# Jiraiya812/Fast-CU-Decision-HEVC

Hardware: AMD Instinct MI355X
Metric: CTUs/sec (RDO decision only) at 4K all-intra (higher is better)
Workload: dtype int32+f64

## Files before the change

### fast-cu-decision-hevc_amd/csrc/fcu_engine.h

```cpp
#pragma once
#include <stdint.h>
#include <string.h>
#include <type_traits>
#include "../../include/fcu.h"

#ifdef FCU_EMU
#include <math.h>
#include <stdio.h>
#include <stdlib.h>
#define FCU_DEV static inline
#define FCU_MEMBER inline
#define FCU_NOINLINE
#define FCU_INLINE
#define FCU_TABLE static const
static int g_emu_phase = 0, g_emu_in_phase = 0, g_emu_lane = 0, g_emu_relax = 0;
#define FCU_EMU_RELAX(on) (g_emu_relax = (on))
static inline int fcu_emu_phase_begin() { g_emu_phase++; g_emu_in_phase = 1; g_emu_lane = 0; return 0; }
static inline int fcu_emu_phase_next(int lane) { if (lane + 1 >= 64) g_emu_in_phase = 0; g_emu_lane = lane + 1; return lane + 1; }
template <class T> static inline T fcu_emu_uni(T v, int site, int line)
{
  enum { SITES = 2048, K = 32, B = 16 };
  struct Seen { int phase, first, cur, idx, n; unsigned char vals[K][B]; };
  static Seen seen[SITES];
  if (g_emu_in_phase && !g_emu_relax && sizeof(T) <= B && site < SITES) {
// ... 3 lines not shown
    if (g_emu_lane == s.first) { if (s.n < K) memcpy(s.vals[s.n++], &v, sizeof(T)); }
    else if (s.idx < s.n && memcmp(s.vals[s.idx], &v, sizeof(T)) != 0) { fprintf(stderr, "FCU_UNI at line %d: value differs between lanes of one phase\n", line); abort(); }
    s.idx++;
  }
  return v;
}
#define FCU_FOR_LANES for (int lane = fcu_emu_phase_begin(); lane < 64; lane = fcu_emu_phase_next(lane))
#define FCU_ATOMIC_ADD(p, v) (*(p) += (v))
#define FCU_ATOMIC_MAX(p, v) do { if (*(p) < (v)) *(p) = (v); } while (0)
#define FCU_ATOMIC_OR(p, v) (*(p) |= (v))
#define FCU_WAVE_ADD(p, v) (*(p) += (v))
#define FCU_WAVE_MIN64(p, v) do { if ((v) < *(p)) *(p) = (v); } while (0)
#define FCU_IN_LDS(p) do { } while (0)
#define FCU_UNI(x) fcu_emu_uni((x), __COUNTER__, __LINE__)
#define FCU_HBM
#define FCU_FLOOR(x) floor(x)
#define FCU_CHECK(c) do { if (!(c)) { fprintf(stderr, "FCU_CHECK failed: %s (line %d)\n", #c, __LINE__); abort(); } } while (0)
static unsigned long long g_emu_cu_paths[3] = { 0, 0, 0 };
#else
#define FCU_DEV __device__ static
#define FCU_MEMBER __device__ inline
#define FCU_NOINLINE __noinline__
#define FCU_INLINE __attribute__((always_inline))
#define FCU_TABLE __device__ static const
#define FCU_FOR_LANES for (int lane = (int)threadIdx.x, fcu_once_ = 1; fcu_once_; fcu_once_ = 0, __syncthreads())
#define FCU_ATOMIC_ADD(p, v) atomicAdd((p), (v))
#define FCU_ATOMIC_MAX(p, v) atomicMax((p), (v))
#define FCU_ATOMIC_OR(p, v) atomicOr((p), (v))
__device__ inline uint32_t fcu_wave_sum(uint32_t v)
{
// ... 17 lines not shown
#define FCU_WAVE_ADD(p, v) do { const uint32_t s_ = fcu_wave_sum(v); if (threadIdx.x == 0) *(p) += s_; } while (0)
#define FCU_WAVE_MIN64(p, v) do { const unsigned long long s_ = fcu_wave_min64(v); if (threadIdx.x == 0 && s_ < *(p)) *(p) = s_; } while (0)
template <class T> __device__ inline T fcu_uni(T v)
{
  static_assert(sizeof(T) % 4 == 0, "dword-sized objects only");
  int w[sizeof(T) / 4];
  __builtin_memcpy(w, &v, sizeof(T));
  for (unsigned i = 0; i < sizeof(T) / 4; i++) w[i] = __builtin_amdgcn_readfirstlane(w[i]);
  __builtin_memcpy(&v, w, sizeof(T));
  return v;
}
#define FCU_UNI(x) fcu_uni(x)
#define FCU_EMU_RELAX(on) do { } while (0)
#if defined(__HIP_DEVICE_COMPILE__)
#define FCU_HBM __attribute__((address_space(1)))
#else
#define FCU_HBM
#endif
#define FCU_GENERIC_(p) ((const __attribute__((address_space(0))) void *)(p))
#define FCU_IN_LDS(p) __builtin_assume(__builtin_amdgcn_is_shared(FCU_GENERIC_(p)))
#define FCU_FLOOR(x) floor(x)
#define FCU_CHECK(c) do { } while (0)
#endif
#define FCU_DIST_ADD(acc, v, e, i, n2) do { \
    if ((n2) >= 64) { (acc) += (uint32_t)((e) * (e)); if (((((i) - lane) + 64) & ((n2) - 1)) == 0) { FCU_WAVE_ADD(&g_S.vc_dist[v], acc); (acc) = 0; } } \
    else FCU_ATOMIC_ADD(&g_S.vc_dist[v], (uint32_t)((e) * (e))); } while (0)
#define FCU_SERIAL FCU_FOR_LANES if (lane == 0)
#if defined(FCU_PROFILE) && !defined(FCU_EMU)
#define FCU_TIC(v) const long long v = clock64()
#ifdef FCU_PROFILE_RQT
#define FCU_QTIC(v) long long v = clock64()
#define FCU_QTOC(E_, v, idx) do { if (threadIdx.x == 0) (E_).C->prof[idx] += (unsigned long long)(clock64() - v); v = clock64(); } while (0)
// ... 4 lines not shown
#define FCU_TOC(E_, v, idx) do { if ((idx) == 10 && threadIdx.x == 0) (E_).C->prof[idx] += (unsigned long long)(clock64() - v); } while (0)
#define FCU_COUNT(E_, idx, n) do { } while (0)
#elif defined(FCU_PROFILE_RDOQ) || defined(FCU_PROFILE_DEPTH)
#define FCU_TOC(E_, v, idx) do { if ((idx) < 11 && threadIdx.x == 0) (E_).C->prof[idx] += (unsigned long long)(clock64() - v); } while (0)
#define FCU_COUNT(E_, idx, n) do { } while (0)
#elif defined(FCU_PROFILE_RMD)
#define FCU_MTOC(E_, v, idx) do { if (threadIdx.x == 0) (E_).C->prof[idx] += (unsigned long long)(clock64() - v); } while (0)
#define FCU_TOC(E_, v, idx) do { if ((idx) < 11 && threadIdx.x == 0) (E_).C->prof[idx] += (unsigned long long)(clock64() - v); } while (0)
#define FCU_COUNT(E_, idx, n) do { } while (0)
#elif defined(FCU_PROFILE_CUSYN)
#define FCU_STOC(E_, v, idx) do { if (threadIdx.x == 0) (E_).C->prof[idx] += (unsigned long long)(clock64() - v); } while (0)
#define FCU_SPATH(E_, path) do { if (threadIdx.x == 0) (E_).C->prof[15] += 1ull << (21 * (path)); } while (0)
#define FCU_S7_COEFF(E_, v, comp) do { if (g_S.prof_s7 == 1) FCU_STOC(E_, v, (comp) ? 14 : 13); } while (0)
#define FCU_TOC(E_, v, idx) do { if ((idx) < 11 && threadIdx.x == 0) (E_).C->prof[idx] += (unsigned long long)(clock64() - v); } while (0)
#define FCU_COUNT(E_, idx, n) do { } while (0)
#else
#define FCU_TOC(E_, v, idx) do { if (threadIdx.x == 0) (E_).C->prof[idx] += (unsigned long long)(clock64() - v); } while (0)
#define FCU_COUNT(E_, idx, n) do { (E_).C->prof[idx] += (unsigned long long)(n); } while (0)
#endif
#else
#define FCU_TIC(v) do { } while (0)
#define FCU_TOC(E_, v, idx) do { } while (0)
#define FCU_COUNT(E_, idx, n) do { } while (0)
#endif
#ifndef FCU_QTOC
#define FCU_QTIC(v) do { } while (0)
#define FCU_QTOC(E_, v, idx) do { } while (0)
#endif
#ifndef FCU_ITOC
#define FCU_ITOC(E_, v, idx) do { } while (0)
#endif
#ifndef FCU_MTOC
#define FCU_MTOC(E_, v, idx) do { } while (0)
#endif
#ifndef FCU_STOC
#define FCU_STOC(E_, v, idx) do { } while (0)
#define FCU_SPATH(E_, path) do { } while (0)
#define FCU_S7_COEFF(E_, v, comp) do { } while (0)
#endif

#include "fcu_tables.h"

struct HotTables { uint32_t bin[256]; uint16_t scan[3][16]; uint8_t scan_cg8[3][4]; uint8_t ctx_ind_map4x4[16]; uint8_t group_idx[32];
                   uint64_t scan4_nib[3], map4_nib; uint32_t cnt_bits[4]; };
#ifdef FCU_EMU
static HotTables g_hot;
#else
__shared__ HotTables g_hot;
// ... 106 lines not shown
  Yuv16 resi_cu, resi_best, qt_resi[4];
  Yuv tmp_pred;
  uint8_t me_pred[9][CTU * CTU];
  int16_t me_h[3][72 * 64];
  int par_ps[4];
  int memo_valid[4][MEMO_K], memo_next[4], memo_zero[4][MEMO_K];
  int16_t memo_mv[4][MEMO_K][NPART][2]; int8_t memo_ref[4][MEMO_K][NPART];
  uint8_t memo_tr_idx[4][MEMO_K][NPART], memo_cbf[4][MEMO_K][3][NPART], memo_tskip[4][MEMO_K][3][NPART];
  alignas(16) int16_t memo_coef[MEMO_K * MEMO_POOL], memo_resi[MEMO_K * MEMO_POOL];
};

struct Env { Chain *C; Scratch *G; int cur_ctu, slice_start; };
struct TU { int log2, tr_depth, part, nparts, x, y, off_y, cw, cwo, cx, cy, c_tr_depth, c_code_all, off_c, cu_depth, plast; };

struct Shared {
  Cabac cab[1 + (MAXDEPTH + 1) + MAXLC + 1];
  uint8_t ref5[5][68]; int dc5[5]; uint32_t cm_dist[5];
  union {
    int16_t lane_abs[MAXLC][32];
    RdoqRec rq_rec[16];
    struct {
      int32_t colsum[128];
      union {
        struct { uint8_t ref[264], reff[264]; };
        uint8_t ref5b[5][68];
      };
    };
  };
  union {
    int16_t rq_lv[16];
    uint32_t sad[36];
// ... 37 lines not shown
  uint64_t lf_frac; uint32_t lf_bins; int lf_valid;
  double dec_j0, dec_j1; int dec_cnt, dec_flip;
#ifdef FCU_PROFILE_CUSYN
  int prof_s7;
#endif
};

enum { CAB_GOON = 0, CAB_CUR0 = 1, CAB_LANE0 = 1 + (MAXDEPTH + 1), CAB_LUMA = CAB_LANE0 + MAXLC };
enum { EST_CODERS = 7 };
static_assert(EST_CODERS * sizeof(Cabac) >= NCTX_INTRA * 2 * sizeof(uint32_t) && EST_CODERS <= MAXLC, "est table does not fit its lane coders");
#define FCU_EST ((uint32_t *)&g_S.cab[CAB_LANE0 + MAXLC - EST_CODERS])
enum { RMD_STAGE_BYTES = 64 * 8 * 2, RMD_COST_BYTES = 35 * 8 };
static_assert(RMD_STAGE_BYTES + RMD_COST_BYTES <= MAXLC * sizeof(Cabac) && (CAB_LANE0 * sizeof(Cabac)) % 8 == 0, "RMD staging does not fit the lane coders");
#define FCU_RMD_STAGE ((int16_t *)&g_S.cab[CAB_LANE0])
#define FCU_RMD_COST ((double *)((char *)&g_S.cab[CAB_LANE0] + RMD_STAGE_BYTES))
FCU_DEV int ref_key(int px, int py, int log2) { return px | (py << 13) | (log2 << 26); }
#ifdef FCU_EMU
static Shared g_S;
#else
__shared__ Shared g_S;
#endif
FCU_DEV Env env_get() { return FCU_UNI(g_S.env); }
FCU_DEV Cabac *slot_ptr(const Env E, int d, int ci) { return ci == CI_CURR_BEST ? &g_S.cab[CAB_CUR0 + d] : &E.G->slots[d][ci]; }


FCU_DEV int part_x(int z) { return (k_z2r[z] & 15) << 2; }
FCU_DEV int part_y(int z) { return (k_z2r[z] >> 4) << 2; }
FCU_DEV int zidx_of(int lx, int ly) { return k_r2z[((ly & 63) >> 2) * 16 + ((lx & 63) >> 2)]; }
FCU_DEV int ilog2(int n) { int l = 0; while ((1 << l) < n) l++; return l; }
FCU_DEV int iabs(int v) { return v < 0 ? -v : v; }
// ... 416 lines not shown
}
FCU_DEV FCU_INLINE int rdoq_signs(const FCU_HBM int32_t *srcg, FCU_HBM int16_t *dstg, int st, int bestLastIdxP1, int lastScanPos)
{
  int absSum = 0;
  for (int sp0 = 0; sp0 < bestLastIdxP1; sp0 += 16) {
    int lv[16]; int32_t sv[16];
#pragma unroll
    for (int k = 0; k < 16; k++) { const int ok = sp0 + k < bestLastIdxP1; lv[k] = ok ? dstg[(sp0 + k) * st] : 0; sv[k] = ok ? srcg[(sp0 + k) * st] : 0; }
#pragma unroll
    for (int k = 0; k < 16; k++) if (sp0 + k < bestLastIdxP1) { absSum += lv[k]; dstg[(sp0 + k) * st] = (int16_t)((sv[k] < 0) ? -lv[k] : lv[k]); }
  }
  for (int sp = bestLastIdxP1; sp <= lastScanPos; sp++) dstg[sp * st] = 0;

  return absSum;
}
FCU_DEV FCU_INLINE void rdoq_sign_hiding(const Params &P, const FCU_HBM int32_t *srcg, FCU_HBM int16_t *dstg, const FCU_HBM RdoqRec *recg, int st, int ch, int bestLastIdxP1, int absSum)
{
  if (P.sign_hiding && absSum >= 2) {
    const long long rdFactor = P.rd_factor[ch];
    int lastCG = -1;
    for (int subSet = (bestLastIdxP1 - 1) >> 4; subSet >= 0; subSet--) {
      const int subPos = subSet << 4; int firstNZ = 16, lastNZ = -1, sum = 0, n;
      uint32_t nzMask = 0, negMask = 0;
      {
        int lv16[16];
#pragma unroll
        for (int k = 0; k < 16; k++) lv16[k] = dstg[(subPos + k) * st];
#pragma unroll
        for (int k = 0; k < 16; k++) { sum += lv16[k]; nzMask |= (uint32_t)(lv16[k] != 0) << k; negMask |= (uint32_t)(lv16[k] < 0) << k; }
      }
      if (nzMask) { lastNZ = 31 - __builtin_clz(nzMask); firstNZ = __builtin_ctz(nzMask); }
// ... 245 lines not shown
template <> struct LaneVar<double> {
  double r = 0;
  __device__ void set(int, double x) { r = x; }
  __device__ double own(int) const { return r; }
  __device__ double get(int k) const
  { union { double d; int i[2]; } u; u.d = r; u.i[0] = FCU_READLANE(u.i[0], k); u.i[1] = FCU_READLANE(u.i[1], k); return u.d; }
  __device__ void put(int k, double x)
  { union { double d; int i[2]; } u, w; u.d = r; w.d = x; u.i[0] = FCU_WRITELANE(w.i[0], k, u.i[0]); u.i[1] = FCU_WRITELANE(w.i[1], k, u.i[1]); r = u.d; }
};
__device__ inline uint32_t lane_mask16(const LaneVar<int> &f) { return (uint32_t)FCU_BALLOT(f.r != 0) & 0xffffu; }
#endif

#ifndef FCU_WAVE_RDOQ_MIN_LOG2
#define FCU_WAVE_RDOQ_MIN_LOG2 2
#endif
FCU_DEV FCU_NOINLINE void rdoq_wave(int c, const int32_t *src, int16_t *dst, int topNZ, int log2, int comp, int scanType, int cbfCtx, const Params &P_, RdoqRec *rec, double *costCGSig)
{
  const Params &P = *FCU_UNI(&P_);
  c = FCU_UNI(c); src = FCU_UNI(src); dst = FCU_UNI(dst); topNZ = FCU_UNI(topNZ); log2 = FCU_UNI(log2); comp = FCU_UNI(comp);
  scanType = FCU_UNI(scanType); cbfCtx = FCU_UNI(cbfCtx); rec = FCU_UNI(rec); costCGSig = FCU_UNI(costCGSig);
  if (topNZ < 0) { FCU_SERIAL { g_S.rw_abs = 0; g_S.rw_lsp = -1; } return; }
  const FCU_HBM int32_t *srcg = (const FCU_HBM int32_t *)src; FCU_HBM int16_t *dstg = (FCU_HBM int16_t *)dst;
  FCU_HBM RdoqRec *recg = (FCU_HBM RdoqRec *)rec; FCU_HBM double *cgg = (FCU_HBM double *)costCGSig;
  auto cb = [&](int ctx, int bin) -> int { return (int)FCU_EST[ctx * 2 + bin]; };
  const int ch = comp ? 1 : 0, N = 1 << log2, n2 = N * N;
  const int qp = comp ? P.qp_c : P.qp;
  const int qbits = rdoq_qbits(log2, qp);
  const double lambda = P.rdoq_lambda[comp];
  const double errScale = P.err_scale[ch][log2 - 2];
  const uint16_t *scan = log2 == 2 ? &g_hot.scan[scanType][0] : k_scan + k_scan_off[scanType * 4 + log2 - 2];
  const uint8_t *scanCG = log2 <= 3 ? g_hot.scan_cg8[log2 == 2 ? 0 : scanType] : k_scan_cg + k_scan_cg_off[scanType * 4 + log2 - 2];
  const int wg = N >> 2, firstSig = first_sig_ctx(log2, scanType, ch);
  const int sigOff = CTX_SIG + (ch ? 28 : 0), cgBase = CTX_SIGCG + (ch ? 2 : 0);
  const uint64_t scan4 = g_hot.scan4_nib[scanType], map4 = g_hot.map4_nib;
  const int cgTop = topNZ >> 4;
  uint64_t cgflag = 0;
  int cgLastScanPos = -1; uint32_t ctxSet = 0; int c1 = 1, c2 = 0;
// ... 349 lines not shown
  int32_t s = 0;
#pragma unroll
  for (int n = 0; n < N; n++) s += (int32_t)(int8_t)(mw[n >> 2] >> (8 * (n & 3))) * (int32_t)a[n];
  return s;
}
template <class F>
FCU_DEV void by_log2(int log2, F f)
{
  switch (log2) {
    case 2: f(std::integral_constant<int, 2>()); break;
    case 3: f(std::integral_constant<int, 3>()); break;
    case 4: f(std::integral_constant<int, 4>()); break;
    default: f(std::integral_constant<int, 5>()); break;
  }
}
template <int LOG2> FCU_DEV const int8_t *basis_row(int useDst, int k) { return (useDst && LOG2 == 2) ? k_dst4 + k * 4 : k_dct + k_dct_off[LOG2 - 2] + (k << LOG2); }
template <int LOG2> FCU_DEV const int8_t *basis_col(int useDst, int n) { return (useDst && LOG2 == 2) ? k_dst4_t + n * 4 : k_dct_t + k_dct_off[LOG2 - 2] + (n << LOG2); }
FCU_DEV int tr_index(int i, int log2) { const int N = 1 << log2; return ((i & (N - 1)) << log2) + (i >> log2); }
template <int LOG2> FCU_DEV int32_t fwd1(const int16_t *resi, int useDst, int idx)
{ constexpr int N = 1 << LOG2, s1 = LOG2 - 1; const int k = idx >> LOG2, y = idx & (N - 1); return (dot_row<N>(basis_row<LOG2>(useDst, k), resi + (y << LOG2)) + (1 << (s1 - 1))) >> s1; }
template <int LOG2> FCU_DEV int32_t fwd2(const int32_t *tmp, int useDst, int idx)
{ constexpr int N = 1 << LOG2, s2 = LOG2 + 6; const int k2 = idx >> LOG2, k1 = idx & (N - 1); return (dot_row<N>(basis_row<LOG2>(useDst, k2), tmp + (k1 << LOG2)) + (1 << (s2 - 1))) >> s2; }
template <int LOG2> FCU_DEV int32_t inv1(const int32_t *deqT, int useDst, int idx)
{ constexpr int N = 1 << LOG2; const int y = idx >> LOG2, kh = idx & (N - 1); return clip3i(-32768, 32767, (dot_row<N>(basis_col<LOG2>(useDst, y), deqT + (kh << LOG2)) + 64) >> 7); }
template <int LOG2> FCU_DEV int32_t inv2(const int32_t *tmp2, int useDst, int idx)
{ constexpr int N = 1 << LOG2; const int y = idx >> LOG2, x = idx & (N - 1); return clip3i(-32768, 32767, (dot_row<N>(basis_col<LOG2>(useDst, x), tmp2 + (y << LOG2)) + 2048) >> 12); }
template <int LOG2> FCU_DEV int32_t fwd1(RowCache<(1 << LOG2), int16_t> &rc, const int16_t *resi, int useDst, int idx)
{ constexpr int N = 1 << LOG2, s1 = LOG2 - 1; const int k = idx >> LOG2, y = idx & (N - 1); return (dot_regs<N>(basis_row<LOG2>(useDst, k), rc.get(resi + (y << LOG2))) + (1 << (s1 - 1))) >> s1; }
template <int LOG2> FCU_DEV int32_t fwd2(RowCache<(1 << LOG2), int32_t> &rc, const int32_t *tmp, int useDst, int idx)
{ constexpr int N = 1 << LOG2, s2 = LOG2 + 6; const int k2 = idx >> LOG2, k1 = idx & (N - 1); return (dot_regs<N>(basis_row<LOG2>(useDst, k2), rc.get(tmp + (k1 << LOG2))) + (1 << (s2 - 1))) >> s2; }
// ... 160 lines not shown
}

FCU_DEV FCU_NOINLINE uint32_t leaf_luma_bits(int c, const CuObj *cu, uint32_t tu_k)
{
  const Env E = env_get(); c = FCU_UNI(c); cu = FCU_UNI(cu); const TU tu = tu_of_key(FCU_UNI(tu_k));
  const int part = tu.part, partSize = cu->part_size[0], log2 = tu.log2;
  cab_reset_bits(c);
  if (part == 0 && E.C->p.slice_type != SLICE_I) { code_skip_flag(E, c, cu, 0); code_pred_mode(c, cu, 0); }
  if (part == 0 && cu->depth[0] == MAXDEPTH) cab_bin(c, partSize == SIZE_2Nx2N, CTX_PARTSIZE);
  if (partSize == SIZE_2Nx2N ? (part == 0) : (tu.tr_depth > 0 && (part & ((cu->nparts >> 2) - 1)) == 0))
    code_luma_dir_bits(c, cu->intra_dir[0][part], g_S.preds);
  if (!(partSize == SIZE_NxN && tu.tr_depth == 0) && log2 != LOG2_MINTU && log2 != min_tu_log2_in_cu(cu->depth[part], cu->part_size[part]))
    cab_bin(c, 0, CTX_SUBDIV + 5 - log2);
  const int cbf = g_S.t_abs > 0;
  cab_bin(c, cbf, CTX_CBF_LUMA + (tu.tr_depth == 0 ? 1 : 0));
  if (cbf) code_coeff_body<1>(c, E.G->p_qscan, 1, g_S.t_lsp, log2, 0, coef_scan_idx(cu->intra_dir[0][part], log2, 0), cu->tskip[0][part], E.C->p, g_S.lane_abs[0]);
  return cab_bits(c);
}

FCU_DEV FCU_NOINLINE void encode_transform(int c, const CuObj *cu, int cuPart, uint32_t root_k, int withLuma)
{
  const Env E = env_get(); c = FCU_UNI(c); cu = FCU_UNI(cu); cuPart = FCU_UNI(cuPart); const TU root = tu_of_key(FCU_UNI(root_k)); withLuma = FCU_UNI(withLuma);
  TU *st = g_S.wk_st; int *ci = g_S.wk_ci; int sp = 0;
  st[0] = root; ci[0] = -1;
  while (sp >= 0) {
    const TU tu = st[sp];
    if (ci[sp] < 0) {
      const int part = cuPart + tu.part, trIdx = tu.tr_depth, subdiv = cu->tr_idx[part] > trIdx;
      if (cu->part_size[part] == SIZE_NxN && trIdx == 0) { }
      else if (tu.log2 > LOG2_MAXTU) { }
      else if (tu.log2 == LOG2_MINTU) { }
// ... 119 lines not shown
  }
}
FCU_DEV FCU_NOINLINE void copy_reco_to_pic(const Yuv *r, int x, int y, int s)
{
  const Env E = env_get(); r = FCU_UNI(r); x = FCU_UNI(x); y = FCU_UNI(y); s = FCU_UNI(s);
  FCU_FOR_LANES {
    for (int c = 0; c < 3; c++) {
      const int sh = c ? 1 : 0, bs = c ? 32 : 64, w = E.C->p.width >> sh, h = E.C->p.height >> sh;
      const uint8_t *src = c == 0 ? r->y : (c == 1 ? r->u : r->v);
      const int px = x >> sh, py = y >> sh, n = s >> sh;
      for (int i = lane; i < n * n; i += 64) { const int yy = i / n, xx = i % n; if (py + yy < h && px + xx < w) E.C->rec[c][(py + yy) * E.C->stride[c] + px + xx] = src[yy * bs + xx]; }
    }
  }
}

FCU_DEV FCU_NOINLINE void tu_trial(CuObj *cu, uint32_t tu_k, int comp, int cab, int save1load2)
{
  const Env E = env_get(); cu = FCU_UNI(cu); const TU tu = tu_of_key(FCU_UNI(tu_k)); comp = FCU_UNI(comp); cab = FCU_UNI(cab); save1load2 = FCU_UNI(save1load2);
  Scratch *G = E.G; const Params &P = E.C->p;
  if (comp && tu.cw == 0) { FCU_SERIAL { g_S.t_dist = 0; g_S.t_abs = 0; g_S.t_lsp = -1; } return; }
  FCU_TIC(t11_);
  const int d = cu->depth_cu, N = comp ? tu.cw : (1 << tu.log2), log2 = ilog2(N), n2 = N * N;
  const int bx = comp ? tu.cx : tu.x, by = comp ? tu.cy : tu.y, bs = comp ? 32 : 64, sh = comp ? 1 : 0;
  const int part = tu.part, layer = LOG2_MAXTU - tu.log2;
  uint8_t *org = yuv_plane(&G->org[d], comp) + by * bs + bx;
  uint8_t *pred = yuv_plane(&G->predt[d], comp) + by * bs + bx;
  uint8_t *recqt = yuv_plane(&G->qt_rec[layer], comp) + by * bs + bx;
  const int px = (cu->x >> sh) + bx, py = (cu->y >> sh) + by;
  uint8_t *recpic = E.C->rec[comp] + py * E.C->stride[comp] + px; const int rs = E.C->stride[comp];
  int16_t *coef = G->qt_coef[comp][layer] + (comp ? tu.off_c : tu.off_y);
  const int useTS = cu->tskip[comp][part];
  const int mode = comp ? chroma_final_mode(cu, part) : cu->intra_dir[0][part];
  const int useDst = comp == 0 && log2 == 2;
  const int qp = comp ? P.qp_c : P.qp;

  if (save1load2 != 2) {
    const int filt = use_filtered_ref(mode, log2, comp == 0);
// ... 13 lines not shown
    FCU_FOR_LANES {
      if (lane == 0) g_S.t_last = -1;
      for (int i = lane; i < n2; i += 64) {
        const int y = i >> log2, x = i & (N - 1); const int v = G->shared_pred[comp][i];
        pred[y * bs + x] = (uint8_t)v; G->p_resi[i] = (int16_t)(org[y * bs + x] - v);
      }
    }
  }
  const int scanType = coef_scan_idx(mode, log2, comp), qbits = rdoq_qbits(log2, qp), qscale = k_quant_scales[qp % 6];
  const uint16_t *iscan = k_iscan + k_scan_off[scanType * 4 + log2 - 2];
  if (useTS) { FCU_FOR_LANES { est_build(cab, lane); for (int i = lane; i < n2; i += 64) { const int sp = iscan[i]; const int32_t ld = level_double((int32_t)G->p_resi[i] << (15 - 8 - log2), qscale, qbits); G->p_lscan[sp] = ld; if (level_nonzero(ld, qbits)) FCU_ATOMIC_MAX(&g_S.t_last, sp); } } }
  else {
    FCU_FOR_LANES { by_log2(log2, [&](auto L) { constexpr int LG = decltype(L)::value; RowCache<(1 << LG), int16_t> rc; for (int i = lane; i < n2; i += 64) G->p_tmp[i] = fwd1<LG>(rc, G->p_resi, useDst, i); }); }
    FCU_FOR_LANES { est_build(cab, lane); by_log2(log2, [&](auto L) { constexpr int LG = decltype(L)::value; RowCache<(1 << LG), int32_t> rc; for (int i = lane; i < n2; i += 64) { const int sp = iscan[i]; const int32_t ld = level_double(fwd2<LG>(rc, G->p_tmp, useDst, i), qscale, qbits); G->p_lscan[sp] = ld; if (level_nonzero(ld, qbits)) FCU_ATOMIC_MAX(&g_S.t_last, sp); } }); }
  }
  {
    FCU_TIC(t8_);
    const int cbfCtx = comp ? (CTX_CBF_CHROMA + tu.tr_depth) : (CTX_CBF_LUMA + (tu.tr_depth == 0 ? 1 : 0));
    const int useRdoq = FCU_UNI((int)(useTS ? P.rdoq_ts : P.rdoq));
    const int onWave = useRdoq && log2 >= FCU_WAVE_RDOQ_MIN_LOG2;
    if (onWave) rdoq_wave(cab, G->p_lscan, G->p_qscan, FCU_UNI(g_S.t_last), log2, comp, scanType, cbfCtx, P, G->r_rec, G->r_cg);
    FCU_FOR_LANES {
      if (comp == 0) for (int i = lane; i < tu.nparts; i += 64) cu->tr_idx[part + i] = (uint8_t)tu.tr_depth;
      if (lane == 0) {
        if (onWave) { g_S.t_abs = g_S.rw_abs; g_S.t_lsp = g_S.rw_lsp; }
        else if (useRdoq) { const RdoqOut o = rdoq<1, 1>(cab, G->p_lscan, G->p_qscan, 1, g_S.t_last, log2, comp, scanType, cbfCtx, P, G->r_rec, G->r_cg); g_S.t_abs = o.abs_sum; g_S.t_lsp = o.last; }
        else { const RdoqOut o = quant_plain(G->p_lscan, G->p_qscan, 1, g_S.t_last, log2, comp, P); g_S.t_abs = o.abs_sum; g_S.t_lsp = o.last; }
        E.C->n_tu_trials++;
        FCU_COUNT(E, 15, (1ull << 40) + (unsigned long long)(g_S.t_last >= 0 ? ((g_S.t_last >> 4) + 1) * 16 : 0));
      }
    }
    FCU_TOC(E, t8_, 8);
  }
  const int absSum = g_S.t_abs;
  FCU_FOR_LANES {
    const int np = comp ? tu_nparts_c(tu) : tu.nparts;
    for (int i = lane; i < np; i += 64) cu->cbf[comp][part + i] = (uint8_t)((absSum > 0 ? 1 : 0) << tu.tr_depth);
    const int cgEnd = ((g_S.t_last >> 4) + 1) << 4;
    const DeqParams dq = deq_params(log2, qp);
    for (int i = lane; i < n2; i += 64) { const int sp = iscan[i]; const int q = (absSum > 0 && sp < cgEnd) ? G->p_qscan[sp] : 0; coef[sp] = (int16_t)q; G->p_tmp[useTS ? i : tr_index(i, log2)] = dequant1(q, dq); }
  }
  if (absSum > 0) {
    if (useTS) { FCU_FOR_LANES { const int s = 15 - 8 - log2; for (int i = lane; i < n2; i += 64) G->p_resi[i] = (int16_t)((G->p_tmp[i] + (1 << (s - 1))) >> s); } }
    else {
      FCU_FOR_LANES { by_log2(log2, [&](auto L) { constexpr int LG = decltype(L)::value; RowCache<(1 << LG), int32_t> rc; for (int i = lane; i < n2; i += 64) G->p_tcoef[i] = inv1<LG>(rc, G->p_tmp, useDst, i); }); }
      FCU_FOR_LANES { by_log2(log2, [&](auto L) { for (int i = lane; i < n2; i += 64) G->p_resi[i] = (int16_t)inv2<decltype(L)::value>(G->p_tcoef, useDst, i); }); }
    }
  }
  FCU_FOR_LANES {
    if (lane == 0) g_S.sad[35] = 0;
  }
  FCU_FOR_LANES {
    uint32_t sse = 0;
    for (int i = lane; i < n2; i += 64) {
      const int y = i >> log2, x = i & (N - 1);
      const int r = clip8(pred[y * bs + x] + (absSum > 0 ? G->p_resi[i] : 0));
      pred[y * bs + x] = (uint8_t)r; recqt[y * bs + x] = (uint8_t)r; recpic[y * rs + x] = (uint8_t)r;
      const int e = org[y * bs + x] - r; sse += (uint32_t)(e * e);
    }
    FCU_WAVE_ADD(&g_S.sad[35], sse);
  }
  FCU_SERIAL { const uint32_t sse = g_S.sad[35]; g_S.t_dist = comp ? (uint32_t)(P.chroma_weight * (double)sse) : sse; }
  FCU_TOC(E, t11_, 11);
}

FCU_DEV FCU_NOINLINE void store_intra_result_qt(uint32_t tu_k, int comp)
{
  const Env E = env_get(); const TU tu = tu_of_key(FCU_UNI(tu_k)); comp = FCU_UNI(comp);
  Scratch *G = E.G;
  if (comp && tu.cw == 0) return;
  const int N = comp ? tu.cw : (1 << tu.log2), layer = LOG2_MAXTU - tu.log2, bs = comp ? 32 : 64, bx = comp ? tu.cx : tu.x, by = comp ? tu.cy : tu.y;
  const int16_t *src = G->qt_coef[comp][layer] + (comp ? tu.off_c : tu.off_y);
  const uint8_t *s = yuv_plane(&G->qt_rec[layer], comp) + by * bs + bx; uint8_t *t = yuv_plane(&G->ts_rec, comp) + by * bs + bx;
  FCU_FOR_LANES { for (int i = lane; i < N * N; i += 64) { G->ts_coef[comp][i] = src[i]; t[(i / N) * bs + (i % N)] = s[(i / N) * bs + (i % N)]; } }
}
FCU_DEV FCU_NOINLINE void load_intra_result_qt(const CuObj *cu, uint32_t tu_k, int comp)
{
// ... 353 lines not shown
}

FCU_DEV FCU_NOINLINE void pu_first_pass_batched(CuObj *cu, uint32_t tu_k)
{
  const Env E = env_get(); cu = FCU_UNI(cu); const TU tu = tu_of_key(FCU_UNI(tu_k));
  Scratch *G = E.G; const Params &P = E.C->p;
  const int d = cu->depth_cu, N = 1 << tu.log2, log2 = tu.log2, n2 = N * N, part = tu.part;
  const int partSize = cu->part_size[part];
  int checkTS = P.transform_skip && log2 == 2;
  if (P.ts_fast) checkTS = checkTS && (partSize == SIZE_NxN);
  const int nc = g_S.n_rd, tsv = checkTS ? 2 : 1, tss = tsv - 1, nvc = nc * tsv;
  FCU_CHECK(nvc <= MAXVC && nvc * n2 <= POOL && (MAXLC % 2) == 0);
  const int qbits = rdoq_qbits(log2, P.qp), qscale = k_quant_scales[P.qp % 6];
  const int useDst = log2 == 2;
  const uint8_t *org = G->org[d].y + tu.y * 64 + tu.x;
  const int haveRefs = FCU_UNI(g_S.ref_tag) == ref_key(cu->x + tu.x, cu->y + tu.y, log2);
  if (!haveRefs) { FCU_TIC(tm_); build_ref(0, cu->x + tu.x, cu->y + tu.y, log2, 1); FCU_MTOC(E, tm_, 14); }
  FCU_FOR_LANES {
    if (lane == 0) g_S.ref_tag = -1;
    const int dc = g_S.dc;
    for (int i = lane; i < nc * n2; i += 64) {
      const int cnd = i / n2, p = i - cnd * n2, y = p >> log2, x = p & (N - 1), mode = g_S.rd_mode[cnd];
      const uint8_t *r = use_filtered_ref(mode, log2, 1) ? g_S.reff : g_S.ref;
      const int v = pred_pixel(r, log2, mode, 1, dc, x, y);
      G->p_pred[i] = (uint8_t)v; G->p_resi[i] = (int16_t)(org[y * 64 + x] - v);
    }
  }
  FCU_FOR_LANES { if (lane < nvc) g_S.vc_last[lane] = -1; by_log2(log2, [&](auto L) { constexpr int LG = decltype(L)::value; RowCache<(1 << LG), int16_t> rc; for (int i = lane; i < nc * n2; i += 64) { const int cnd = i / n2; G->p_tmp[i] = fwd1<LG>(rc, G->p_resi + cnd * n2, useDst, i - cnd * n2); } }); }
  FCU_FOR_LANES {
    est_build(CAB_CUR0 + d, lane);
    by_log2(log2, [&](auto L) { constexpr int LG = decltype(L)::value; RowCache<(1 << LG), int32_t> rc;
      for (int i = lane; i < nvc * n2; i += 64) {
        const int v = i / n2, p = i - v * n2, cnd = (v >> tss), ts = (v & tss);
        const uint16_t *iscan = k_iscan + k_scan_off[coef_scan_idx(g_S.rd_mode[cnd], log2, 0) * 4 + log2 - 2];
        const int32_t t = ts ? ((int32_t)G->p_resi[cnd * n2 + p] << (15 - 8 - log2)) : fwd2<LG>(rc, G->p_tmp + cnd * n2, useDst, p);
        const int sp = iscan[p]; const int32_t ld = level_double(t, qscale, qbits);
        G->p_lscan[sp * nvc + v] = ld;
        if (level_nonzero(ld, qbits)) FCU_ATOMIC_MAX(&g_S.vc_last[v], sp);
      }
    });
  }
  FCU_TIC(t2_);
  FCU_FOR_LANES {
    if (lane < nvc) {
      const int mode = g_S.rd_mode[(lane >> tss)];
      RdoqRec *rrec = G->r_rec + lane; double *rcg = G->r_cg + lane;
      const int cbfCtx = CTX_CBF_LUMA + (tu.tr_depth == 0 ? 1 : 0);
      const RdoqOut o = ((lane & tss) ? P.rdoq_ts : P.rdoq) ? rdoq<0, 1>(CAB_CUR0 + d, G->p_lscan + lane, G->p_qscan + lane, nvc, g_S.vc_last[lane], log2, 0, coef_scan_idx(mode, log2, 0), cbfCtx, P, rrec, rcg)
                                                            : quant_plain(G->p_lscan + lane, G->p_qscan + lane, nvc, g_S.vc_last[lane], log2, 0, P);
      g_S.vc_abs[lane] = o.abs_sum; g_S.vc_lsp[lane] = o.last;
      g_S.vc_dist[lane] = 0;
    }
    if (lane == 0) E.C->n_tu_trials += (unsigned long long)nvc;
  }
  FCU_TOC(E, t2_, 2);
  FCU_FOR_LANES {
    const DeqParams dq = deq_params(log2, P.qp);
    for (int i = lane; i < nvc * n2; i += 64) {
      const int v = i / n2, p = i - v * n2;
      const uint16_t *iscan = k_iscan + k_scan_off[coef_scan_idx(g_S.rd_mode[(v >> tss)], log2, 0) * 4 + log2 - 2];
      const int sp = iscan[p];
      const int q = (g_S.vc_abs[v] > 0 && (sp >> 4) <= (g_S.vc_last[v] >> 4)) ? G->p_qscan[sp * nvc + v] : 0;
      G->p_tmp[((v & tss)) ? i : v * n2 + tr_index(p, log2)] = dequant1(q, dq);
    }
  }
  FCU_FOR_LANES {
    by_log2(log2, [&](auto L) { constexpr int LG = decltype(L)::value; RowCache<(1 << LG), int32_t> rc;
      for (int i = lane; i < nvc * n2; i += 64) {
        const int v = i / n2, p = i - v * n2, ts = (v & tss);
        if (ts) { const int s = 15 - 8 - log2; G->p_tcoef[i] = (G->p_tmp[i] + (1 << (s - 1))) >> s; }
// ... 3 lines not shown
  }
  FCU_FOR_LANES {
    by_log2(log2, [&](auto L) {
      uint32_t acc = 0;
      for (int i = lane; i < nvc * n2; i += 64) {
        const int v = i / n2, p = i - v * n2, cnd = (v >> tss), ts = (v & tss), y = p >> log2, x = p & (N - 1);
        int res = 0;
        if (g_S.vc_abs[v] > 0) res = ts ? (int16_t)G->p_tcoef[i] : inv2<decltype(L)::value>(G->p_tcoef + v * n2, useDst, p);
        const int r = clip8(G->p_pred[cnd * n2 + p] + res);
        G->p_rec[i] = (uint8_t)r;
        const int e = org[y * 64 + x] - r;
        FCU_DIST_ADD(acc, v, e, i, n2);
      }
    });
  }
  FCU_TIC(t3_);
  for (int vbase = 0; vbase < nvc; vbase += MAXLC) {
    const int slotBase = vbase ? (g_S.vc_slot[g_S.pu_best_vc] + 1) % MAXLC : 0;
#if defined(FCU_EMU) && defined(FCU_EMU_TRACE_ROUNDS)
    if (vbase) fprintf(stderr, "second bit-count round: %d variants\n", nvc);
#endif
    FCU_FOR_LANES {
      const int vc = vbase + lane;
      if (lane < MAXLC && vc < nvc) {
        const int cnd = (vc >> tss), ts = (vc & tss), mode = g_S.rd_mode[cnd], cbf = g_S.vc_abs[vc] > 0;
        const int slot = (slotBase + lane) % MAXLC;
        double cost;
        g_S.vc_slot[vc] = (uint8_t)slot;
        if (ts && !cbf) cost = FCU_MAX_DOUBLE;
        else {
// ... 319 lines not shown
  const int d = cu->depth_cu;
  const int N = tu.cw, log2 = ilog2(N), n2 = N * N, trDepth = tu.tr_depth;
  int checkTS = P.transform_skip && N <= 4;
  if (P.ts_fast) {
    checkTS = checkTS && (tu.log2 == 2);
    if (checkTS) { int nb = 0; const int maxp = tu.part + (tu.c_code_all ? 1 : 4); for (int p = tu.part; p < maxp; p++) nb += cu->tskip[0][p]; checkTS = checkTS && (nb > 0); }
  }
  const int tsv = checkTS ? 2 : 1, tss = tsv - 1;
  const int perRound = (tsv == 1 && 10 * n2 <= POOL) ? 2 : 1;
  const int nm = 5 * perRound, nvc = nm * tsv;
  const int qbits = rdoq_qbits(log2, P.qp_c), qscale = k_quant_scales[P.qp_c % 6];
  const int subPart = tu_part_c(tu), nPartsC = tu_nparts_c(tu);
  const int lumaDir = cu->intra_dir[0][tu.part & ~3];
  for (int comp0 = 1; comp0 < 3; comp0 += perRound) {
    const int px = (cu->x >> 1) + tu.cx, py = (cu->y >> 1) + tu.cy;
    for (int cc = 0; cc < perRound; cc++) {
      const int comp = comp0 + cc;
      const uint8_t *org = yuv_plane(&G->org[d], comp) + tu.cy * 32 + tu.cx;
      chroma_leaf_refs5(E, cu, comp, px, py, log2);
      FCU_FOR_LANES {
        for (int i = lane; i < 5 * n2; i += 64) {
          const int m = i / n2, p = i - m * n2, y = p >> log2, x = p & (N - 1);
          const int mode = g_S.c_modes[m] == DM_CHROMA ? lumaDir : g_S.c_modes[m];
          const int pr = pred_pixel(g_S.ref5[m], log2, mode, 0, g_S.dc5[m], x, y);
          G->p_pred[cc * 5 * n2 + i] = (uint8_t)pr; G->p_resi[cc * 5 * n2 + i] = (int16_t)(org[y * 32 + x] - pr);
        }
      }
    }
    FCU_FOR_LANES { if (lane < nvc) g_S.vc_last[lane] = -1; by_log2(log2, [&](auto L) { constexpr int LG = decltype(L)::value; RowCache<(1 << LG), int16_t> rc; for (int i = lane; i < nm * n2; i += 64) { const int b = i / n2; G->p_tmp[i] = fwd1<LG>(rc, G->p_resi + b * n2, 0, i - b * n2); } }); }
    FCU_FOR_LANES {
      by_log2(log2, [&](auto L) { constexpr int LG = decltype(L)::value; RowCache<(1 << LG), int32_t> rc;
        for (int i = lane; i < nvc * n2; i += 64) {
          const int v = i / n2, p = i - v * n2, b = (v >> tss), ts = (v & tss), m = b % 5, comp = comp0 + b / 5;
          const int mode = g_S.c_modes[m] == DM_CHROMA ? lumaDir : g_S.c_modes[m];
          const uint16_t *iscan = k_iscan + k_scan_off[coef_scan_idx(mode, log2, comp) * 4 + log2 - 2];
          const int32_t t = ts ? ((int32_t)G->p_resi[b * n2 + p] << (15 - 8 - log2)) : fwd2<LG>(rc, G->p_tmp + b * n2, 0, p);
          const int sp = iscan[p]; const int32_t ld = level_double(t, qscale, qbits);
          G->p_lscan[sp * nvc + v] = ld;
          if (level_nonzero(ld, qbits)) FCU_ATOMIC_MAX(&g_S.vc_last[v], sp);
        }
      });
    }
    FCU_TIC(t13_);
    FCU_FOR_LANES {
      if (lane < nvc) {
        const int b = (lane >> tss), m = b % 5, comp = comp0 + b / 5;
        const int mode = g_S.c_modes[m] == DM_CHROMA ? lumaDir : g_S.c_modes[m];
        RdoqRec *rrec = G->r_rec + lane; double *rcg = G->r_cg + lane;
        const RdoqOut o = ((lane & tss) ? P.rdoq_ts : P.rdoq)
          ? rdoq<0, 0>(CAB_LANE0 + m, G->p_lscan + lane, G->p_qscan + lane, nvc, g_S.vc_last[lane], log2, 1 , coef_scan_idx(mode, log2, comp), CTX_CBF_CHROMA + trDepth, P, rrec, rcg)
          : quant_plain(G->p_lscan + lane, G->p_qscan + lane, nvc, g_S.vc_last[lane], log2, 1, P);
        g_S.vc_abs[lane] = o.abs_sum; g_S.vc_lsp[lane] = o.last;
        g_S.vc_dist[lane] = 0;
      }
      if (lane == 0) E.C->n_tu_trials += (unsigned long long)nvc;
    }
    FCU_TOC(E, t13_, 13);
    FCU_FOR_LANES {
      const DeqParams dq = deq_params(log2, P.qp_c);
      for (int i = lane; i < nvc * n2; i += 64) {
        const int v = i / n2, p = i - v * n2, b = (v >> tss), m = b % 5, comp = comp0 + b / 5;
        const int mode = g_S.c_modes[m] == DM_CHROMA ? lumaDir : g_S.c_modes[m];
        const uint16_t *iscan = k_iscan + k_scan_off[coef_scan_idx(mode, log2, comp) * 4 + log2 - 2];
        const int sp = iscan[p];
        const int q = (g_S.vc_abs[v] > 0 && (sp >> 4) <= (g_S.vc_last[v] >> 4)) ? G->p_qscan[sp * nvc + v] : 0;
        G->p_tmp[((v & tss)) ? i : v * n2 + tr_index(p, log2)] = dequant1(q, dq);
      }
    }
    FCU_FOR_LANES {
      by_log2(log2, [&](auto L) { constexpr int LG = decltype(L)::value; RowCache<(1 << LG), int32_t> rc;
        for (int i = lane; i < nvc * n2; i += 64) {
          const int v = i / n2, p = i - v * n2, ts = (v & tss);
// ... 5 lines not shown
    FCU_FOR_LANES {
      by_log2(log2, [&](auto L) {
        uint32_t acc = 0;
        for (int i = lane; i < nvc * n2; i += 64) {
          const int v = i / n2, p = i - v * n2, b = (v >> tss), ts = (v & tss), y = p >> log2, x = p & (N - 1);
          const uint8_t *org = yuv_plane(&G->org[d], comp0 + b / 5) + tu.cy * 32 + tu.cx;
          int res = 0;
          if (g_S.vc_abs[v] > 0) res = ts ? (int16_t)G->p_tcoef[i] : inv2<decltype(L)::value>(G->p_tcoef + v * n2, 0, p);
          const int r = clip8(G->p_pred[b * n2 + p] + res);
          G->p_rec[i] = (uint8_t)r;
          const int e = org[y * 32 + x] - r;
          FCU_DIST_ADD(acc, v, e, i, n2);
        }
      });
    }
    FCU_FOR_LANES {
      if (lane < 5) {
        const int m = lane; int bestTs = 0;
        const int mode = g_S.c_modes[m] == DM_CHROMA ? lumaDir : g_S.c_modes[m];
        if (tsv == 2) {
          const int comp = comp0;
          uint32_t dsel = (uint32_t)(P.chroma_weight * (double)g_S.vc_dist[m * 2]);
          const uint32_t d0 = dsel, d1 = (uint32_t)(P.chroma_weight * (double)g_S.vc_dist[m * 2 + 1]);
          const int c0 = CAB_LANE0 + 5 + m, c1 = CAB_LANE0 + 10 + m;
          cab_copy1(&g_S.cab[c0], &g_S.cab[CAB_LANE0 + m]); cab_reset_bits(c0);
          if (g_S.vc_abs[m * 2] > 0) code_coeff_nxn<0>(c0, G->p_qscan + m * 2, nvc, g_S.vc_lsp[m * 2], log2, comp, coef_scan_idx(mode, log2, comp), 0, P, g_S.lane_abs[lane]);
          const double cost0 = rd_cost(P, cab_bits(c0), d0);
          double cost1 = FCU_MAX_DOUBLE;
          if (g_S.vc_abs[m * 2 + 1] > 0) {
            cab_copy1(&g_S.cab[c1], &g_S.cab[CAB_LANE0 + m]); cab_reset_bits(c1);
// ... 584 lines not shown
```

Before: 19910.

## Add LDS-staged fast path for small luma TU trials with wave RDOQ

Adds tu_trial_small, a dedicated path for 4x4/8x8 luma TU trials that stages prediction, residual, transform, quantized-level and reconstruction buffers in LDS (aliased over the lane CABAC coders) instead of global scratch. It also templates rdoq_wave and the sign-hiding helper so they can use LDS address-space pointers. Coefficients are written straight into qt_coef, and the bit-counting path now reads from there. The intent is to cut global-memory traffic and per-element loop overhead on very frequent small TUs; the cost is aliasing LDS that the coders use, which requires the staging to stay disjoint from live coder state. Profiling hooks for small-TU sections are added but compile out by default.

```diff
diff --git a/fast-cu-decision-hevc_amd/csrc/fcu_engine.h b/fast-cu-decision-hevc_amd/csrc/fcu_engine.h
--- a/fast-cu-decision-hevc_amd/csrc/fcu_engine.h
+++ b/fast-cu-decision-hevc_amd/csrc/fcu_engine.h
@@ -41,6 +41,7 @@
 #define FCU_IN_LDS(p) do { } while (0)
 #define FCU_UNI(x) fcu_emu_uni((x), __COUNTER__, __LINE__)
 #define FCU_HBM
+#define FCU_LDS
 #define FCU_FLOOR(x) floor(x)
 #define FCU_CHECK(c) do { if (!(c)) { fprintf(stderr, "FCU_CHECK failed: %s (line %d)\n", #c, __LINE__); abort(); } } while (0)
 static unsigned long long g_emu_cu_paths[3] = { 0, 0, 0 };
@@ -88,8 +89,10 @@
 #define FCU_EMU_RELAX(on) do { } while (0)
 #if defined(__HIP_DEVICE_COMPILE__)
 #define FCU_HBM __attribute__((address_space(1)))
+#define FCU_LDS __attribute__((address_space(3)))
 #else
 #define FCU_HBM
+#define FCU_LDS
 #endif
 #define FCU_GENERIC_(p) ((const __attribute__((address_space(0))) void *)(p))
 #define FCU_IN_LDS(p) __builtin_assume(__builtin_amdgcn_is_shared(FCU_GENERIC_(p)))
@@ -124,6 +127,14 @@
 #define FCU_S7_COEFF(E_, v, comp) do { if (g_S.prof_s7 == 1) FCU_STOC(E_, v, (comp) ? 14 : 13); } while (0)
 #define FCU_TOC(E_, v, idx) do { if ((idx) < 11 && threadIdx.x == 0) (E_).C->prof[idx] += (unsigned long long)(clock64() - v); } while (0)
 #define FCU_COUNT(E_, idx, n) do { } while (0)
+#elif defined(FCU_PROFILE_SMALLTU)
+#define FCU_ZCLS(log2_) ((log2_) <= 2 ? 0 : (log2_) == 3 ? 1 : 2)
+#define FCU_ZTIC(v) long long v = clock64()
+#define FCU_ZRE(v) (v = clock64())
+#define FCU_ZTOC(E_, v, sec, log2_) do { if (threadIdx.x == 0) (E_).C->prof[(sec) * 3 + FCU_ZCLS(log2_)] += (unsigned long long)(clock64() - v); } while (0)
+#define FCU_ZCNT(E_, sec, log2_) do { if (threadIdx.x == 0) (E_).C->prof[11 + (sec)] += 1ull << (21 * FCU_ZCLS(log2_)); } while (0)
+#define FCU_TOC(E_, v, idx) do { if ((idx) == 10 && threadIdx.x == 0) (E_).C->prof[idx] += (unsigned long long)(clock64() - v); } while (0)
+#define FCU_COUNT(E_, idx, n) do { } while (0)
 #else
 #define FCU_TOC(E_, v, idx) do { if (threadIdx.x == 0) (E_).C->prof[idx] += (unsigned long long)(clock64() - v); } while (0)
 #define FCU_COUNT(E_, idx, n) do { (E_).C->prof[idx] += (unsigned long long)(n); } while (0)
@@ -142,6 +153,12 @@
 #endif
 #ifndef FCU_MTOC
 #define FCU_MTOC(E_, v, idx) do { } while (0)
+#endif
+#ifndef FCU_ZTOC
+#define FCU_ZTIC(v) do { } while (0)
+#define FCU_ZRE(v) do { } while (0)
+#define FCU_ZTOC(E_, v, sec, log2_) do { } while (0)
+#define FCU_ZCNT(E_, sec, log2_) do { } while (0)
 #endif
 #ifndef FCU_STOC
 #define FCU_STOC(E_, v, idx) do { } while (0)
@@ -278,7 +295,7 @@
 struct TU { int log2, tr_depth, part, nparts, x, y, off_y, cw, cwo, cx, cy, c_tr_depth, c_code_all, off_c, cu_depth, plast; };
 
 struct Shared {
-  Cabac cab[1 + (MAXDEPTH + 1) + MAXLC + 1];
+  alignas(16) Cabac cab[1 + (MAXDEPTH + 1) + MAXLC + 1];
   uint8_t ref5[5][68]; int dc5[5]; uint32_t cm_dist[5];
   union {
     int16_t lane_abs[MAXLC][32];
@@ -346,6 +363,9 @@
 static_assert(RMD_STAGE_BYTES + RMD_COST_BYTES <= MAXLC * sizeof(Cabac) && (CAB_LANE0 * sizeof(Cabac)) % 8 == 0, "RMD staging does not fit the lane coders");
 #define FCU_RMD_STAGE ((int16_t *)&g_S.cab[CAB_LANE0])
 #define FCU_RMD_COST ((double *)((char *)&g_S.cab[CAB_LANE0] + RMD_STAGE_BYTES))
+struct SmallTu { int32_t tmp[64], lscan[64], tcoef[64]; int16_t resi[64], qscan[64]; uint8_t pred[64], org[64], sp[64]; };
+static_assert(sizeof(SmallTu) <= (MAXLC - EST_CODERS) * sizeof(Cabac) && (CAB_LANE0 * sizeof(Cabac)) % 16 == 0, "small-TU staging does not fit the lane coders below the est table");
+#define FCU_SMALLTU ((SmallTu *)&g_S.cab[CAB_LANE0])
 FCU_DEV int ref_key(int px, int py, int log2) { return px | (py << 13) | (log2 << 26); }
 #ifdef FCU_EMU
 static Shared g_S;
@@ -792,7 +812,8 @@
 
   return absSum;
 }
-FCU_DEV FCU_INLINE void rdoq_sign_hiding(const Params &P, const FCU_HBM int32_t *srcg, FCU_HBM int16_t *dstg, const FCU_HBM RdoqRec *recg, int st, int ch, int bestLastIdxP1, int absSum)
+template <class SrcP, class DstP, class RecP>
+FCU_DEV FCU_INLINE void rdoq_sign_hiding(const Params &P, SrcP srcg, DstP dstg, RecP recg, int st, int ch, int bestLastIdxP1, int absSum)
 {
   if (P.sign_hiding && absSum >= 2) {
     const long long rdFactor = P.rd_factor[ch];
@@ -1068,13 +1089,16 @@
 #ifndef FCU_WAVE_RDOQ_MIN_LOG2
 #define FCU_WAVE_RDOQ_MIN_LOG2 2
 #endif
+template <int LDSIO = 0>
 FCU_DEV FCU_NOINLINE void rdoq_wave(int c, const int32_t *src, int16_t *dst, int topNZ, int log2, int comp, int scanType, int cbfCtx, const Params &P_, RdoqRec *rec, double *costCGSig)
 {
   const Params &P = *FCU_UNI(&P_);
   c = FCU_UNI(c); src = FCU_UNI(src); dst = FCU_UNI(dst); topNZ = FCU_UNI(topNZ); log2 = FCU_UNI(log2); comp = FCU_UNI(comp);
   scanType = FCU_UNI(scanType); cbfCtx = FCU_UNI(cbfCtx); rec = FCU_UNI(rec); costCGSig = FCU_UNI(costCGSig);
   if (topNZ < 0) { FCU_SERIAL { g_S.rw_abs = 0; g_S.rw_lsp = -1; } return; }
-  const FCU_HBM int32_t *srcg = (const FCU_HBM int32_t *)src; FCU_HBM int16_t *dstg = (FCU_HBM int16_t *)dst;
+  typedef typename std::conditional<LDSIO != 0, const FCU_LDS int32_t *, const FCU_HBM int32_t *>::type SrcP;
+  typedef typename std::conditional<LDSIO != 0, FCU_LDS int16_t *, FCU_HBM int16_t *>::type DstP;
+  SrcP srcg = (SrcP)src; DstP dstg = (DstP)dst;
   FCU_HBM RdoqRec *recg = (FCU_HBM RdoqRec *)rec; FCU_HBM double *cgg = (FCU_HBM double *)costCGSig;
   auto cb = [&](int ctx, int bin) -> int { return (int)FCU_EST[ctx * 2 + bin]; };
   const int ch = comp ? 1 : 0, N = 1 << log2, n2 = N * N;
@@ -1454,6 +1478,8 @@
     default: f(std::integral_constant<int, 5>()); break;
   }
 }
+template <class F>
+FCU_DEV void by_log2_small(int log2, F f) { if (log2 == 2) f(std::integral_constant<int, 2>()); else f(std::integral_constant<int, 3>()); }
 template <int LOG2> FCU_DEV const int8_t *basis_row(int useDst, int k) { return (useDst && LOG2 == 2) ? k_dst4 + k * 4 : k_dct + k_dct_off[LOG2 - 2] + (k << LOG2); }
 template <int LOG2> FCU_DEV const int8_t *basis_col(int useDst, int n) { return (useDst && LOG2 == 2) ? k_dst4_t + n * 4 : k_dct_t + k_dct_off[LOG2 - 2] + (n << LOG2); }
 FCU_DEV int tr_index(int i, int log2) { const int N = 1 << log2; return ((i & (N - 1)) << log2) + (i >> log2); }
@@ -1644,7 +1670,7 @@
     cab_bin(c, 0, CTX_SUBDIV + 5 - log2);
   const int cbf = g_S.t_abs > 0;
   cab_bin(c, cbf, CTX_CBF_LUMA + (tu.tr_depth == 0 ? 1 : 0));
-  if (cbf) code_coeff_body<1>(c, E.G->p_qscan, 1, g_S.t_lsp, log2, 0, coef_scan_idx(cu->intra_dir[0][part], log2, 0), cu->tskip[0][part], E.C->p, g_S.lane_abs[0]);
+  if (cbf) code_coeff_body<1>(c, E.G->qt_coef[0][LOG2_MAXTU - log2] + tu.off_y, 1, g_S.t_lsp, log2, 0, coef_scan_idx(cu->intra_dir[0][part], log2, 0), cu->tskip[0][part], E.C->p, g_S.lane_abs[0]);
   return cab_bits(c);
 }
 
@@ -1794,13 +1820,107 @@
   }
 }
 
+FCU_DEV FCU_NOINLINE void tu_trial_small(CuObj *cu, uint32_t tu_k, int cab, int save1load2)
+{
+  const Env E = env_get(); cu = FCU_UNI(cu); const TU tu = tu_of_key(FCU_UNI(tu_k)); cab = FCU_UNI(cab); save1load2 = FCU_UNI(save1load2);
+  Scratch *G = E.G; const Params &P = E.C->p;
+  FCU_TIC(t11_);
+  const int d = cu->depth_cu, log2 = tu.log2, N = 1 << log2, n2 = N * N;
+  FCU_ZTIC(tz_); FCU_ZCNT(E, 0, log2);
+  const int part = tu.part, layer = LOG2_MAXTU - log2;
+  const uint8_t *org = G->org[d].y + tu.y * 64 + tu.x;
+  uint8_t *pred = G->predt[d].y + tu.y * 64 + tu.x;
+  uint8_t *recqt = G->qt_rec[layer].y + tu.y * 64 + tu.x;
+  const int px = cu->x + tu.x, py = cu->y + tu.y;
+  uint8_t *recpic = E.C->rec[0] + py * E.C->stride[0] + px; const int rs = E.C->stride[0];
+  int16_t *coef = G->qt_coef[0][layer] + tu.off_y;
+  const int useTS = cu->tskip[0][part], mode = cu->intra_dir[0][part], useDst = log2 == 2, qp = P.qp;
+  const int filt = use_filtered_ref(mode, log2, 1);
+  SmallTu *S = FCU_SMALLTU;
+  FCU_CHECK(log2 <= 3 && (useTS ? P.rdoq_ts : P.rdoq));
+
+  if (save1load2 != 2) build_ref(0, px, py, log2, filt);
+  FCU_FOR_LANES {
+    if (lane == 0) g_S.t_last = -1;
+    if (lane < n2) {
+      const int y = lane >> log2, x = lane & (N - 1);
+      int v;
+      if (save1load2 != 2) {
+        v = pred_pixel(filt ? g_S.reff : g_S.ref, log2, mode, 1, g_S.dc, x, y);
+        if (save1load2 == 1) G->shared_pred[0][lane] = (uint8_t)v;
+      } else v = G->shared_pred[0][lane];
+      const int o = org[y * 64 + x];
+      S->pred[lane] = (uint8_t)v; S->org[lane] = (uint8_t)o; S->resi[lane] = (int16_t)(o - v);
+    }
+  }
+  const int scanType = coef_scan_idx(mode, log2, 0), qbits = rdoq_qbits(log2, qp), qscale = k_quant_scales[qp % 6];
+  const uint16_t *iscan = k_iscan + k_scan_off[scanType * 4 + log2 - 2];
+  if (useTS) {
+    FCU_FOR_LANES {
+      est_build(cab, lane);
+      if (lane < n2) { const int sp = iscan[lane]; const int32_t ld = level_double((int32_t)S->resi[lane] << (15 - 8 - log2), qscale, qbits); S->sp[lane] = (uint8_t)sp; S->lscan[sp] = ld; if (level_nonzero(ld, qbits)) FCU_ATOMIC_MAX(&g_S.t_last, sp); }
+    }
+  } else {
+    FCU_FOR_LANES { est_build(cab, lane); if (lane < n2) by_log2_small(log2, [&](auto L) { S->tmp[lane] = fwd1<decltype(L)::value>(S->resi, useDst, lane); }); }
+    FCU_FOR_LANES {
+      if (lane < n2) by_log2_small(log2, [&](auto L) {
+        const int sp = iscan[lane]; const int32_t ld = level_double(fwd2<decltype(L)::value>(S->tmp, useDst, lane), qscale, qbits);
+        S->sp[lane] = (uint8_t)sp; S->lscan[sp] = ld; if (level_nonzero(ld, qbits)) FCU_ATOMIC_MAX(&g_S.t_last, sp);
+      });
+    }
+  }
+  FCU_ZTOC(E, tz_, 0, log2);
+  {
+    FCU_TIC(t8_);
+    rdoq_wave<1>(cab, S->lscan, S->qscan, FCU_UNI(g_S.t_last), log2, 0, scanType, CTX_CBF_LUMA + (tu.tr_depth == 0 ? 1 : 0), P, G->r_rec, G->r_cg);
+    FCU_TOC(E, t8_, 8);
+  }
+  FCU_ZRE(tz_);
+  const int absSum = FCU_UNI(g_S.rw_abs);
+  FCU_FOR_LANES {
+    for (int i = lane; i < tu.nparts; i += 64) { cu->tr_idx[part + i] = (uint8_t)tu.tr_depth; cu->cbf[0][part + i] = (uint8_t)((absSum > 0 ? 1 : 0) << tu.tr_depth); }
+    if (lane == 0) {
+      g_S.t_abs = absSum; g_S.t_lsp = g_S.rw_lsp; g_S.sad[35] = 0;
+      E.C->n_tu_trials++;
+      FCU_COUNT(E, 15, (1ull << 40) + (unsigned long long)(g_S.t_last >= 0 ? ((g_S.t_last >> 4) + 1) * 16 : 0));
+    }
+    if (lane < n2) {
+      const int cgEnd = ((g_S.t_last >> 4) + 1) << 4;
+      const DeqParams dq = deq_params(log2, qp);
+      const int sp = S->sp[lane]; const int q = (absSum > 0 && sp < cgEnd) ? S->qscan[sp] : 0;
+      coef[sp] = (int16_t)q; S->tmp[useTS ? lane : tr_index(lane, log2)] = dequant1(q, dq);
+    }
+  }
+  if (absSum > 0 && !useTS) FCU_FOR_LANES { if (lane < n2) by_log2_small(log2, [&](auto L) { S->tcoef[lane] = inv1<decltype(L)::value>(S->tmp, useDst, lane); }); }
+  FCU_FOR_LANES {
+    uint32_t sse = 0;
+    if (lane < n2) {
+      const int y = lane >> log2, x = lane & (N - 1);
+      int res = 0;
+      if (absSum > 0) {
+        if (useTS) { const int s = 15 - 8 - log2; res = (int16_t)((S->tmp[lane] + (1 << (s - 1))) >> s); }
+        else by_log2_small(log2, [&](auto L) { res = (int16_t)inv2<decltype(L)::value>(S->tcoef, useDst, lane); });
+      }
+      const int r = clip8(S->pred[lane] + res);
+      pred[y * 64 + x] = (uint8_t)r; recqt[y * 64 + x] = (uint8_t)r; recpic[y * rs + x] = (uint8_t)r;
+      const int e = S->org[lane] - r; sse = (uint32_t)(e * e);
+    }
+    FCU_WAVE_ADD(&g_S.sad[35], sse);
+  }
+  FCU_SERIAL { g_S.t_dist = g_S.sad[35]; }
+  FCU_ZTOC(E, tz_, 0, log2);
+  FCU_TOC(E, t11_, 11);
+}
+
 FCU_DEV FCU_NOINLINE void tu_trial(CuObj *cu, uint32_t tu_k, int comp, int cab, int save1load2)
 {
   const Env E = env_get(); cu = FCU_UNI(cu); const TU tu = tu_of_key(FCU_UNI(tu_k)); comp = FCU_UNI(comp); cab = FCU_UNI(cab); save1load2 = FCU_UNI(save1load2);
   Scratch *G = E.G; const Params &P = E.C->p;
   if (comp && tu.cw == 0) { FCU_SERIAL { g_S.t_dist = 0; g_S.t_abs = 0; g_S.t_lsp = -1; } return; }
+  if (FCU_WAVE_RDOQ_MIN_LOG2 <= 2 && comp == 0 && tu.log2 <= 3 && FCU_UNI((int)(cu->tskip[0][tu.part] ? P.rdoq_ts : P.rdoq))) { tu_trial_small(cu, tu_k, cab, save1load2); return; }
   FCU_TIC(t11_);
   const int d = cu->depth_cu, N = comp ? tu.cw : (1 << tu.log2), log2 = ilog2(N), n2 = N * N;
+  FCU_ZTIC(tz_); FCU_ZCNT(E, 0, log2);
   const int bx = comp ? tu.cx : tu.x, by = comp ? tu.cy : tu.y, bs = comp ? 32 : 64, sh = comp ? 1 : 0;
   const int part = tu.part, layer = LOG2_MAXTU - tu.log2;
   uint8_t *org = yuv_plane(&G->org[d], comp) + by * bs + bx;
@@ -1844,6 +1964,7 @@
     FCU_FOR_LANES { by_log2(log2, [&](auto L) { constexpr int LG = decltype(L)::value; RowCache<(1 << LG), int16_t> rc; for (int i = lane; i < n2; i += 64) G->p_tmp[i] = fwd1<LG>(rc, G->p_resi, useDst, i); }); }
     FCU_FOR_LANES { est_build(cab, lane); by_log2(log2, [&](auto L) { constexpr int LG = decltype(L)::value; RowCache<(1 << LG), int32_t> rc; for (int i = lane; i < n2; i += 64) { const int sp = iscan[i]; const int32_t ld = level_double(fwd2<LG>(rc, G->p_tmp, useDst, i), qscale, qbits); G->p_lscan[sp] = ld; if (level_nonzero(ld, qbits)) FCU_ATOMIC_MAX(&g_S.t_last, sp); } }); }
   }
+  FCU_ZTOC(E, tz_, 0, log2);
   {
     FCU_TIC(t8_);
     const int cbfCtx = comp ? (CTX_CBF_CHROMA + tu.tr_depth) : (CTX_CBF_LUMA + (tu.tr_depth == 0 ? 1 : 0));
@@ -1862,6 +1983,7 @@
     }
     FCU_TOC(E, t8_, 8);
   }
+  FCU_ZRE(tz_);
   const int absSum = g_S.t_abs;
   FCU_FOR_LANES {
     const int np = comp ? tu_nparts_c(tu) : tu.nparts;
@@ -1891,6 +2013,7 @@
     FCU_WAVE_ADD(&g_S.sad[35], sse);
   }
   FCU_SERIAL { const uint32_t sse = g_S.sad[35]; g_S.t_dist = comp ? (uint32_t)(P.chroma_weight * (double)sse) : sse; }
+  FCU_ZTOC(E, tz_, 0, log2);
   FCU_TOC(E, t11_, 11);
 }
 
@@ -2274,6 +2397,7 @@
   const int qbits = rdoq_qbits(log2, P.qp), qscale = k_quant_scales[P.qp % 6];
   const int useDst = log2 == 2;
   const uint8_t *org = G->org[d].y + tu.y * 64 + tu.x;
+  FCU_ZTIC(tz_); FCU_ZCNT(E, 1, log2);
   const int haveRefs = FCU_UNI(g_S.ref_tag) == ref_key(cu->x + tu.x, cu->y + tu.y, log2);
   if (!haveRefs) { FCU_TIC(tm_); build_ref(0, cu->x + tu.x, cu->y + tu.y, log2, 1); FCU_MTOC(E, tm_, 14); }
   FCU_FOR_LANES {
@@ -2300,6 +2424,7 @@
       }
     });
   }
+  FCU_ZTOC(E, tz_, 1, log2);
   FCU_TIC(t2_);
   FCU_FOR_LANES {
     if (lane < nvc) {
@@ -2314,6 +2439,7 @@
     if (lane == 0) E.C->n_tu_trials += (unsigned long long)nvc;
   }
   FCU_TOC(E, t2_, 2);
+  FCU_ZRE(tz_);
   FCU_FOR_LANES {
     const DeqParams dq = deq_params(log2, P.qp);
     for (int i = lane; i < nvc * n2; i += 64) {
@@ -2347,6 +2473,7 @@
       }
     });
   }
+  FCU_ZTOC(E, tz_, 1, log2);
   FCU_TIC(t3_);
   for (int vbase = 0; vbase < nvc; vbase += MAXLC) {
     const int slotBase = vbase ? (g_S.vc_slot[g_S.pu_best_vc] + 1) % MAXLC : 0;
@@ -2696,6 +2823,7 @@
   const int lumaDir = cu->intra_dir[0][tu.part & ~3];
   for (int comp0 = 1; comp0 < 3; comp0 += perRound) {
     const int px = (cu->x >> 1) + tu.cx, py = (cu->y >> 1) + tu.cy;
+    FCU_ZTIC(tz_); FCU_ZCNT(E, 2, log2);
     for (int cc = 0; cc < perRound; cc++) {
       const int comp = comp0 + cc;
       const uint8_t *org = yuv_plane(&G->org[d], comp) + tu.cy * 32 + tu.cx;
@@ -2723,6 +2851,7 @@
         }
       });
     }
+    FCU_ZTOC(E, tz_, 2, log2);
     FCU_TIC(t13_);
     FCU_FOR_LANES {
       if (lane < nvc) {
@@ -2738,6 +2867,7 @@
       if (lane == 0) E.C->n_tu_trials += (unsigned long long)nvc;
     }
     FCU_TOC(E, t13_, 13);
+    FCU_ZRE(tz_);
     FCU_FOR_LANES {
       const DeqParams dq = deq_params(log2, P.qp_c);
       for (int i = lane; i < nvc * n2; i += 64) {
@@ -2773,6 +2903,7 @@
         }
       });
     }
+    FCU_ZTOC(E, tz_, 2, log2);
     FCU_FOR_LANES {
       if (lane < 5) {
         const int m = lane; int bestTs = 0;
```

Result: no change. 19930, median of 2 (+0.1%).
